# IST-DASLab/qutlass

Measured on AMD Instinct MI355X. Metric: TFLOP/s & %FP4-MFMA-peak, MXFP4 GEMM 4096x4096x4096, 1 MI355X, higher is better.
Workload: dtype fp4 (e2m1 x e2m1, e8m0 block scales, fp32 accumulate, bf16 out); 1 GPU; matmul_mxf4_bf16_tn 4096x4096x4096, gs=32 e8m0 scales (BASELINE.json configs[1]); parallelism=single GPU, clock_ramp=8200 untimed steps (~250 ms) before the 5 warmup steps

## Files before the change

qutlass_amd/csrc/capi.hip:

```cpp
#include <hip/hip_runtime.h>

#include <algorithm>
#include <atomic>
#include <chrono>
#include <cmath>
#include <cstdarg>
#include <cstdio>
#include <cstring>

#include "../../include/qutlass_amd.h"
#include "gemm_mx.hip.h"
#include "gemm_mx_deepp.hip.h"
#if QAMD_BENCH
#include "lab/gemm_mx_duo.hip.h"
#include "lab/gemm_mx_deepp_lab.hip.h"
#endif
#include "gemm_mx_skinny.hip.h"
#include "gemm_mx_ks.hip.h"
#include "gemm_mx_os.hip.h"
#include "gemm_mx_os_w4a8.hip.h"
#include "gemm_mx_fusedq.hip.h"
#include "gemm_nvf4.hip.h"
#include "gemm_nvf4_pk.hip.h"
#include "gemm_nvf4_os.hip.h"
#include "quantize.hip.h"
#include "moe_route.hip.h"
#include "to_blocked.hip.h"
#include "transpose_u8.hip.h"
#include "quartet_bwd.hip.h"
#if QAMD_BENCH
#include "lab/quartet_bwd_lab.hip.h"
#endif

using namespace qamd;

#ifndef QAMD_TU
#define QAMD_TU 0
#endif
#define QAMD_DEF(n) (QAMD_TU == 0 || QAMD_TU == (n))
#ifndef QAMD_BENCH
#define QAMD_BENCH 0
#endif

namespace qamd_host {

#if QAMD_DEF(1)
thread_local char g_err[512] = "";
#if QAMD_BENCH
std::atomic<int> g_hw_fp4_cvt{1};
std::atomic<int> g_gemm_variant{0};
std::atomic<int> g_nvf4_variant{0};
std::atomic<int> g_splitk_wg{0};
std::atomic<int> g_splitk_min_kt{32};
std::atomic<int> g_transpose_nc{0};
std::atomic<int> g_pp_shift{2};
std::atomic<int> g_pp_flags{1};
std::atomic<int> g_quant_wg_per_cu{0};
std::atomic<int> g_deepp_grid{0};
std::atomic<int> g_bwd_variant{0};
std::atomic<int> g_moe_sort_one_launch_max{0};
std::atomic<int> g_splitk_force{0};
std::atomic<uint32_t*> g_dbg{nullptr};
#endif

int fail(int code, const char* fmt, ...) {
  va_list ap;
  va_start(ap, fmt);
  vsnprintf(g_err, sizeof(g_err), fmt, ap);
  va_end(ap);
  return code;
}

int check_launch(const char* what) {
  hipError_t e = hipGetLastError();
  if (e != hipSuccess) return fail(QAMD_ERR_HIP, "%s: %s", what, hipGetErrorString(e));
  return QAMD_OK;
}

unsigned long long next_launch_tag() {
  static std::atomic<unsigned long long> tag{[] {
    unsigned long long x = (unsigned long long)std::chrono::steady_clock::now().time_since_epoch().count() ^ ((unsigned long long)(uintptr_t)&g_err << 17);
    x ^= x >> 31; x *= 0x9e3779b97f4a7c15ull; x ^= x >> 29;
    return x | 1ull;
  }()};
  return tag.fetch_add(1, std::memory_order_relaxed) + 1;
}
#else
unsigned long long next_launch_tag();
#if QAMD_BENCH
extern std::atomic<int> g_hw_fp4_cvt, g_gemm_variant, g_nvf4_variant, g_splitk_wg, g_splitk_min_kt, g_transpose_nc, g_pp_shift, g_pp_flags, g_quant_wg_per_cu, g_splitk_force, g_deepp_grid, g_bwd_variant, g_moe_sort_one_launch_max;
extern std::atomic<uint32_t*> g_dbg;
#endif
int fail(int code, const char* fmt, ...);
int check_launch(const char* what);
#endif

#if QAMD_BENCH
inline bool opt_hw_fp4() { return g_hw_fp4_cvt.load() != 0; }
inline int opt_gemm_variant() { return g_gemm_variant.load(); }
inline int opt_nvf4_variant() { return g_nvf4_variant.load(); }
inline int opt_splitk_wg() { return g_splitk_wg.load(); }
inline int opt_splitk_min_kt() { return g_splitk_min_kt.load(); }
inline int opt_transpose_nc() { return g_transpose_nc.load(); }
inline int opt_pp_shift() { return g_pp_shift.load(); }
inline int opt_pp_flags() { return g_pp_flags.load(); }
inline int opt_quant_wg_per_cu() { return g_quant_wg_per_cu.load(); }
inline int opt_splitk_force() { return g_splitk_force.load(); }
inline int opt_deepp_grid() { return g_deepp_grid.load(); }
inline int opt_bwd_variant() { return g_bwd_variant.load(); }
inline int opt_moe_sort_one_launch_max() { return g_moe_sort_one_launch_max.load(); }
inline uint32_t* opt_dbg() { return g_dbg.load(); }
#else
constexpr bool opt_hw_fp4() { return true; }
constexpr int opt_gemm_variant() { return 0; }
constexpr int opt_nvf4_variant() { return 0; }
constexpr int opt_splitk_wg() { return 0; }
constexpr int opt_splitk_min_kt() { return 32; }
constexpr int opt_transpose_nc() { return 0; }
constexpr int opt_pp_shift() { return 2; }
constexpr int opt_pp_flags() { return 1; }
constexpr int opt_quant_wg_per_cu() { return 0; }
constexpr int opt_splitk_force() { return 0; }
constexpr int opt_deepp_grid() { return 0; }
constexpr int opt_bwd_variant() { return 0; }
constexpr int opt_moe_sort_one_launch_max() { return 0; }
constexpr uint32_t* opt_dbg() { return nullptr; }
#endif

inline int64_t cdiv(int64_t a, int64_t b) { return (a + b - 1) / b; }

#if QAMD_DEF(1)
int chip_cus() {
  static std::atomic<int> cache[64];
  int dev = 0;
  if (hipGetDevice(&dev) != hipSuccess || dev < 0 || dev >= 64) return 256;
  int v = cache[dev].load(std::memory_order_relaxed);
  if (v <= 0) {
    int n = 0;
    if (hipDeviceGetAttribute(&n, hipDeviceAttributeMultiprocessorCount, dev) != hipSuccess || n <= 0) n = 256;
    cache[dev].store(n, std::memory_order_relaxed);
    v = n;
  }
  return v;
}
#else
int chip_cus();
#endif


template <class C, int PP>
int launch_gemm(GemmParams p, hipStream_t s) {
  p.tiles_m = (int)cdiv(p.M, C::BM);
  p.tiles_n = (int)cdiv(p.N, C::BN);
  p.raster_magic = raster_magic(p.tiles_n);
  if (PP != 7 && PP != 9) { p.ws = nullptr; p.splits = 1; p.ctr = nullptr; p.tag = 0; }
  hipLaunchKernelGGL((gemm_mx_kernel<C, PP>), dim3(p.tiles_m * p.tiles_n, p.splits), dim3(C::THREADS), 0, s, p);
  return check_launch("gemm_mx_kernel");
}

inline int deepp_grid(int tiles) {
  const int forced = opt_deepp_grid();
  if (forced > 0) return std::min(forced, tiles);
  const int cus = chip_cus();
  const int rounds = (tiles + cus - 1) / cus;
  const int g = ((tiles + rounds - 1) / rounds + 7) / 8 * 8;
  return std::min(std::min(g, cus), tiles);
}

template <class C, bool TRACE = false, int ST_AUX = 0, int LAB = 0>
int launch_gemm_deepp(GemmParams p, hipStream_t s) {
  p.tiles_m = (int)cdiv(p.M, C::BM);
  p.tiles_n = (int)cdiv(p.N, C::BN);
  p.raster_magic = raster_magic(p.tiles_n);
  p.ws = nullptr; p.splits = 1; p.ctr = nullptr; p.tag = 0;
  const int grid = deepp_grid(p.tiles_m * p.tiles_n);
#if QAMD_BENCH
#ifdef QAMD_ROUTE_LABK
  if constexpr (!TRACE && LAB == 0) {
    hipLaunchKernelGGL((labk::gemm_mx_deepp_kernel<C, false, ST_AUX, 8>), dim3(grid), dim3(C::THREADS), 0, s, p);
    return check_launch("labk::gemm_mx_deepp_kernel");
  }
#endif
  if constexpr (TRACE || LAB != 0) {
    hipLaunchKernelGGL((labk::gemm_mx_deepp_kernel<C, TRACE, ST_AUX, LAB>), dim3(grid), dim3(C::THREADS), 0, s, p);
    return check_launch("labk::gemm_mx_deepp_kernel");
  }
#else
  static_assert(!TRACE && LAB == 0, "traces / ablations: lab build only");
#endif
  const int64_t kt = cdiv((int64_t)p.K * C::EBITS / 8, 128);
  const bool odd = (kt & 1) && kt >= 3, one = grid == p.tiles_m * p.tiles_n;
  if (odd && one) hipLaunchKernelGGL((gemm_mx_deepp_kernel<C, ST_AUX, true, true>), dim3(grid), dim3(C::THREADS), 0, s, p);
  else if (odd) hipLaunchKernelGGL((gemm_mx_deepp_kernel<C, ST_AUX, true, false>), dim3(grid), dim3(C::THREADS), 0, s, p);
  else if (one) hipLaunchKernelGGL((gemm_mx_deepp_kernel<C, ST_AUX, false, true>), dim3(grid), dim3(C::THREADS), 0, s, p);
  else hipLaunchKernelGGL((gemm_mx_deepp_kernel<C, ST_AUX>), dim3(grid), dim3(C::THREADS), 0, s, p);
  return check_launch("gemm_mx_deepp_kernel");
}

#if QAMD_BENCH
template <class C, int ST_AUX = 17, int RET = 0, bool TRACE = false>
int launch_gemm_duo(GemmParams p, hipStream_t s) {
  p.tiles_m = (int)cdiv(p.M, C::BM);
  p.tiles_n = (int)cdiv(p.N, C::BN);
  p.raster_magic = raster_magic(p.tiles_n);
  p.ws = nullptr; p.splits = 1; p.ctr = nullptr; p.tag = 0;
  const int grid = deepp_grid(p.tiles_m * p.tiles_n);
  hipLaunchKernelGGL((gemm_mx_duo_kernel<C, ST_AUX, RET, TRACE>), dim3(grid), dim3(C::THREADS), 0, s, p);
  return check_launch("gemm_mx_duo_kernel");
}
#endif

template <int TM, int TN, int D = 8>
int launch_gemm_ks(GemmParams p, hipStream_t s) {
  using C = KsCfg<TM, TN, D>;
  p.tiles_m = (int)cdiv(p.M, TM);
  p.tiles_n = (int)cdiv(p.N, TN);
  p.ws = nullptr; p.splits = 1; p.ctr = nullptr; p.tag = 0;
  hipLaunchKernelGGL((gemm_mx_ks_kernel<C>), dim3(p.tiles_m * p.tiles_n), dim3(256), 0, s, p);
  return check_launch("gemm_mx_ks_kernel");
}

template <bool RM = false, int TN = 32, int EBITS = 4, int TM = 32, int AFMT = 0>
int launch_gemm_os(GemmParams p, hipStream_t s) {
  p.tiles_m = (int)cdiv(p.M, TM);
  p.tiles_n = (int)cdiv(p.N, TN);
  p.ws = nullptr; p.splits = 1; p.ctr = nullptr; p.tag = 0;
  const int64_t KT = cdiv((int64_t)p.K * EBITS / 8, 128);
  const dim3 grid(p.tiles_m * p.tiles_n), block(256);
  constexpr int SMAX = TM == 32 ? 4 : 3;
  if (KT <= 4) hipLaunchKernelGGL((gemm_mx_os_kernel<OsCfg<1, TN, EBITS, TM, AFMT>, RM>), grid, block, 0, s, p);
  else if (KT <= 8) hipLaunchKernelGGL((gemm_mx_os_kernel<OsCfg<2, TN, EBITS, TM, AFMT>, RM>), grid, block, 0, s, p);
  else if (KT <= 12) hipLaunchKernelGGL((gemm_mx_os_kernel<OsCfg<3, TN, EBITS, TM, AFMT>, RM>), grid, block, 0, s, p);
  else if (KT <= 4 * SMAX) hipLaunchKernelGGL((gemm_mx_os_kernel<OsCfg<SMAX, TN, EBITS, TM, AFMT>, RM>), grid, block, 0, s, p);
  else hipLaunchKernelGGL((gemm_mx_os_kernel<OsCfg<SMAX, TN, EBITS, TM, AFMT>, RM, true>), grid, block, 0, s, p);
  return check_launch("gemm_mx_os_kernel");
}
template <int EBITS = 4, int AFMT = 0, bool RM = false, int TN = 16>
int launch_gemm_os16(GemmParams p, hipStream_t s) {
  p.tiles_m = (int)cdiv(p.M, 16);
  p.tiles_n = (int)cdiv(p.N, TN);
  p.ws = nullptr; p.splits = 1; p.ctr = nullptr; p.tag = 0;
  const int64_t KT = cdiv((int64_t)p.K * EBITS / 8, 128);
  const dim3 grid(p.tiles_m * p.tiles_n), block(256);
  constexpr int STAGE = Os16Cfg<1, EBITS, AFMT, TN>::STAGE;
  constexpr int SFIT = 160 * 1024 / (4 * STAGE), SMAX = SFIT >= 8 ? 8 : SFIT >= 4 ? 4 : SFIT;
  static_assert(SMAX >= 3, "LDS budget");
  if (KT <= 4) hipLaunchKernelGGL((gemm_mx_os16_kernel<Os16Cfg<1, EBITS, AFMT, TN>, false, RM>), grid, block, 0, s, p);
  else if (KT <= 8) hipLaunchKernelGGL((gemm_mx_os16_kernel<Os16Cfg<2, EBITS, AFMT, TN>, false, RM>), grid, block, 0, s, p);
  else if (KT <= 16 && SMAX >= 4) hipLaunchKernelGGL((gemm_mx_os16_kernel<Os16Cfg<(SMAX >= 4 ? 4 : SMAX), EBITS, AFMT, TN>, false, RM>), grid, block, 0, s, p);
  else if (KT <= 4 * SMAX) hipLaunchKernelGGL((gemm_mx_os16_kernel<Os16Cfg<SMAX, EBITS, AFMT, TN>, false, RM>), grid, block, 0, s, p);
  else hipLaunchKernelGGL((gemm_mx_os16_kernel<Os16Cfg<SMAX, EBITS, AFMT, TN>, true, RM>), grid, block, 0, s, p);
  return check_launch("gemm_mx_os16_kernel");
}
inline int os16_tn(int64_t N, int64_t cus) {
  for (int tn : {16, 32, 48, 56, 64})
    if (cdiv(N, tn) <= cus) return tn;
  return 0;
}
inline int os16_wide_plan(int ebits, int64_t N, int64_t K, int64_t cus) {
  const int tn = os16_tn(N, cus);
  const int64_t KT = cdiv(K * ebits / 8, 128);
  if (ebits == 4) {
    if (tn == 32) return (KT >= 12 && KT <= 32) ? 572 : 0;
    if (tn == 48) return (KT >= 8 && KT <= 24) ? 573 : 0;
    if (tn == 56) return (KT >= 8 && KT <= 16) ? 574 : 0;
    if (tn == 64) return (KT >= 8 && KT <= 16) ? 575 : 0;
    return 0;
  }
  if (tn == 32) return (KT >= 16 && KT <= 64) ? 572 : 0;
  if (tn == 48) return (KT >= 16 && KT <= 32) ? 573 : 0;
  return 0;
}
template <int EBITS, int AFMT, bool RM>
int launch_gemm_os16_tn(int tn, const GemmParams& p, hipStream_t s) {
  switch (tn) {
    case 16: return launch_gemm_os16<EBITS, AFMT, RM, 16>(p, s);
    case 32: return launch_gemm_os16<EBITS, AFMT, RM, 32>(p, s);
    case 48: return launch_gemm_os16<EBITS, AFMT, RM, 48>(p, s);
    case 56: return launch_gemm_os16<EBITS, AFMT, RM, 56>(p, s);
    case 64: return launch_gemm_os16<EBITS, AFMT, RM, 64>(p, s);
  }
  return fail(QAMD_ERR_INVALID, "gemm_mx_os16: no column tile of %d", tn);
}
inline int os_plan(int64_t M, int64_t N, int64_t K, int64_t cus, bool ada = false) {
  const int64_t T32 = cdiv(M, 32) * cdiv(N, 32), T16 = cdiv(M, 32) * cdiv(N, 16), KT = cdiv(K, 256);
  if (T32 > cus) return 0;
  const int tn = T16 <= cus ? 16 : 32;
  if (KT <= 16) return tn;
  if (KT <= 32) return 4 * T32 >= cus ? tn : 0;
  if (KT > 64 || 2 * T32 < cus) return 0;
  return (ada || M >= 8 || tn == 16) ? tn : 0;
}

inline bool os64_plan(int64_t M, int64_t N, int64_t K, int64_t cus, bool ada = false) {
  const int64_t T32 = cdiv(M, 32) * cdiv(N, 32), T64 = cdiv(M, 64) * cdiv(N, 32), KT = cdiv(K, 256);
  if (T32 <= cus || T64 > cus) return false;
  if (ada) return KT <= 64;
  return KT <= 12 || (KT >= 40 && KT <= 64) || (KT >= 32 && KT < 40 && T64 == cus && M <= 64);
}
inline int os8_plan(int64_t M, int64_t N, int64_t K, int64_t cus) {
  const int64_t T32 = cdiv(M, 32) * cdiv(N, 32), T16 = cdiv(M, 32) * cdiv(N, 16), T64 = cdiv(M, 64) * cdiv(N, 32), KT = cdiv(K, 128);
  if (M <= 16) {
    if (const int v = os16_wide_plan(8, N, K, cus)) return v;
  }
  if (T32 <= cus) {
    const int v = T16 <= cus ? 569 : 568;
    const int64_t G = T16 <= cus ? T16 : T32;
    const bool d16 = cdiv(M, 16) * cdiv(N, 16) <= cus;
    if (KT <= 40) return d16 ? 571 : v;
    if (4 * G < 3 * cus) return 0;
    if (KT <= 64) return d16 ? 571 : v;
    if (KT <= 128) return (M <= 32 || N >= 4096) ? v : 0;
    return (KT <= 256 && M <= 32) ? v : 0;
  }
  return (T64 <= cus && KT > 16 && KT <= 128) ? 570 : 0;
}

inline int grouped_plan(int64_t M, int64_t N, int64_t K, int64_t E, int cus) {
  (void)N; (void)cus;
  return (M <= 32 * E && K <= 1024) ? 590 : 593;
}
inline int64_t grouped_grid(const GroupedFormat& F, int v, int64_t M, int64_t N, int64_t E) {
  return grouped_workgroups(M, N, E, F.tile[v - F.form0].tm, F.tile[v - F.form0].tn);
}
template <const GroupedFormat& F, int I, int AFMT = 0>
int launch_grouped_os(GroupedParams q, hipStream_t s) {
  constexpr int TM = F.tile[I].tm, TN = F.tile[I].tn, EBITS = F.ebits;
  q.tiles_m = 1;
  q.tiles_n = (int)cdiv(q.N, TN);
  const int64_t KT = cdiv((int64_t)q.K * EBITS / 8, 128);
  const dim3 grid((int)grouped_workgroups(q.M, q.N, q.E, TM, TN)), block(256);
  constexpr int SMAX = TM == 32 ? 4 : 3;
  if (KT <= 4) hipLaunchKernelGGL((gemm_mx_os_kernel<OsCfg<1, TN, EBITS, TM, AFMT>, true, false, true>), grid, block, 0, s, q);
  else if (KT <= 8) hipLaunchKernelGGL((gemm_mx_os_kernel<OsCfg<2, TN, EBITS, TM, AFMT>, true, false, true>), grid, block, 0, s, q);
  else if (KT <= 12) hipLaunchKernelGGL((gemm_mx_os_kernel<OsCfg<3, TN, EBITS, TM, AFMT>, true, false, true>), grid, block, 0, s, q);
  else if (KT <= 4 * SMAX) hipLaunchKernelGGL((gemm_mx_os_kernel<OsCfg<SMAX, TN, EBITS, TM, AFMT>, true, false, true>), grid, block, 0, s, q);
  else hipLaunchKernelGGL((gemm_mx_os_kernel<OsCfg<SMAX, TN, EBITS, TM, AFMT>, true, true, true>), grid, block, 0, s, q);
  return check_launch("gemm_mx_os_kernel (grouped)");
}
template <const GroupedFormat& F, class C>
int launch_grouped_ring(GroupedParams q, hipStream_t s) {
  static_assert(C::BM == F.tile[3].tm && C::BN == F.tile[3].tn && C::EBITS == F.ebits, "the ring configuration is the format's fourth form");
  q.tiles_m = 1;
  q.tiles_n = (int)cdiv(q.N, C::BN);
  hipLaunchKernelGGL((gemm_mx_grouped_ring_kernel<C>), dim3((int)grouped_workgroups(q.M, q.N, q.E, C::BM, C::BN)), dim3(C::THREADS), 0, s, q);
  return check_launch("gemm_mx_grouped_ring_kernel");
}
// ... 92 lines not shown
  return check_launch("gemm_mx_deepp_kernel (stream-K)");
}
#endif

template <class C, bool NN = false, int NNABL = 0>
int launch_gemm_deepp8(GemmParams p, hipStream_t s) {
  p.tiles_m = (int)cdiv(p.M, C::BM);
  p.tiles_n = (int)cdiv(p.N, C::BN);
  p.raster_magic = raster_magic(p.tiles_n);
  p.ws = nullptr; p.splits = 1; p.ctr = nullptr; p.tag = 0;
  const int grid = deepp_grid(p.tiles_m * p.tiles_n);
#if QAMD_BENCH
  if constexpr (NNABL != 0) {
    hipLaunchKernelGGL((labk::gemm_mx_deepp8_kernel<C, 17, NN, NNABL>), dim3(grid), dim3(C::THREADS), 0, s, p);
    return check_launch("labk::gemm_mx_deepp8_kernel");
  }
#else
  static_assert(NNABL == 0, "ablations: lab build only");
#endif
  if (grid == p.tiles_m * p.tiles_n) hipLaunchKernelGGL((gemm_mx_deepp8_kernel<C, 17, NN, true>), dim3(grid), dim3(C::THREADS), 0, s, p);
  else hipLaunchKernelGGL((gemm_mx_deepp8_kernel<C, 17, NN>), dim3(grid), dim3(C::THREADS), 0, s, p);
  return check_launch("gemm_mx_deepp8_kernel");
}

template <class CB, class CT, int ST_AUX>
int launch_gemm_hetero(GemmParams p, hipStream_t s) {
  p.tiles_m = (int)cdiv(p.M, CB::BM);
  p.tiles_n = (int)cdiv(p.N, CB::BN);
  p.raster_magic = raster_magic(p.tiles_n);
  p.ws = nullptr; p.splits = 1; p.ctr = nullptr; p.tag = 0;
  const int T = p.tiles_m * p.tiles_n;
  const int forced = opt_deepp_grid();
  const int g_big = std::min(forced > 0 ? forced : chip_cus(), T);
  const int t_main = T / g_big * g_big;
  const int nsmall = 4 * (T - t_main);
  if (nsmall == 0) {
    if constexpr (CB::EBITS == 4) return launch_gemm_deepp<CB, false, ST_AUX>(p, s);
    else return launch_gemm_deepp8<CB>(p, s);
  }
  if constexpr (CB::EBITS == 4) {
    if (const int64_t kt = cdiv((int64_t)p.K, 256); (kt & 1) && kt >= 3) {
      hipLaunchKernelGGL((gemm_mx_hetero_kernel<CB, CT, ST_AUX, true>), dim3(g_big + nsmall), dim3(256), 0, s, p, g_big, t_main);
      return check_launch("gemm_mx_hetero_kernel (odd stage count)");
    }
  }
  hipLaunchKernelGGL((gemm_mx_hetero_kernel<CB, CT, ST_AUX>), dim3(g_big + nsmall), dim3(256), 0, s, p, g_big, t_main);
  return check_launch("gemm_mx_hetero_kernel");
}

inline bool hetero_wins(int64_t T, int cus) {
  const int64_t r = T / cus, rem = T % cus;
  if (r < 1 || rem == 0) return false;
  const int64_t R = r + 1;
  const double a = (double)R * std::max(0.45 + 0.55 * (double)T / (double)(R * cus), 0.78);
  const int64_t nsmall = 4 * rem, waves = nsmall / cus;
  const double last = (double)(nsmall % cus) / (double)cus;
  const double b = (double)r + 0.05 + 0.38 * (double)waves + (last > 0 ? 0.25 + 0.13 * last : 0.0);
  return b < a;
}

#if QAMD_BENCH
#if QAMD_DEF(6)
int dispatch_ablation_mx4(int v, const GemmParams& p, hipStream_t s) {
  switch (v) {
#define QAMD_ABL(b) \
    case 100 + b: return launch_gemm<GemmCfg<256, 256, 2, 4, 4, false, b>, 1>(p, s); \
    case 200 + b: return launch_gemm<GemmCfg<256, 256, 2, 4, 4, false, b>, 0>(p, s); \
    case 300 + b: return launch_gemm<GemmCfg<256, 256, 2, 4, 4, false, b>, 2>(p, s);
    QAMD_ABL(1) QAMD_ABL(2) QAMD_ABL(3) QAMD_ABL(4) QAMD_ABL(8) QAMD_ABL(9) QAMD_ABL(10) QAMD_ABL(11) QAMD_ABL(16) QAMD_ABL(17) QAMD_ABL(18) QAMD_ABL(41) QAMD_ABL(40) QAMD_ABL(42)
#undef QAMD_ABL
  }
  return -1;
}
#else
int dispatch_ablation_mx4(int v, const GemmParams& p, hipStream_t s);
#endif
#endif

template <int EBITS, bool SPLIT>
int dispatch_variant(int v, const GemmParams& p, hipStream_t s, const char* name) {
#if QAMD_BENCH
  if (p.pp_flags & 4096) {
    if (v >= 70 && v <= 73) v += 100;
    else if (v == 24 || v == 25 || (v >= 27 && v <= 29)) v += 200;
  }
#endif
  switch (v) {
    case 24: return launch_gemm<GemmCfg<128, 128, 2, 2, EBITS, SPLIT, 0, 2>, 9>(p, s);
    case 25: return launch_gemm<GemmCfg<256, 128, 4, 2, EBITS, SPLIT, 0, 2>, 9>(p, s);
    case 27: return launch_gemm<GemmCfg<128, 64, 2, 2, EBITS, SPLIT, 0, 2>, 9>(p, s);
    case 58: return launch_gemm<GemmCfg<256, 128, 2, 2, EBITS, SPLIT, 0, 3>, 9>(p, s);
    case 28: return launch_gemm<GemmCfg<64, 128, 2, 2, EBITS, SPLIT, 0, 2>, 9>(p, s);
    case 29: return launch_gemm<GemmCfg<64, 64, 2, 2, EBITS, SPLIT, 0, 2>, 9>(p, s);
    case 70: return launch_gemm<GemmCfg<64, 64, 2, 2, EBITS, SPLIT, 0, 3>, 9>(p, s);
    case 71: return launch_gemm<GemmCfg<128, 64, 2, 2, EBITS, SPLIT, 0, 3>, 9>(p, s);
    case 72: return launch_gemm<GemmCfg<64, 128, 2, 2, EBITS, SPLIT, 0, 3>, 9>(p, s);
    case 73: return launch_gemm<GemmCfg<128, 128, 2, 2, EBITS, SPLIT, 0, 3>, 9>(p, s);
#if QAMD_BENCH
    case 273: return launch_gemm<GemmCfg<128, 128, 2, 2, EBITS, SPLIT, 128, 3>, 9>(p, s);
    case 272: return launch_gemm<GemmCfg<64, 128, 2, 2, EBITS, SPLIT, 128, 3>, 9>(p, s);
    case 270: return launch_gemm<GemmCfg<64, 64, 2, 2, EBITS, SPLIT, 128, 3>, 9>(p, s);
    case 224 + 1000: return launch_gemm<GemmCfg<128, 128, 2, 2, EBITS, SPLIT, 128, 2>, 9>(p, s);
    case 373: return launch_gemm<GemmCfg<128, 128, 2, 4, EBITS, SPLIT, 0, 3>, 9>(p, s);
    case 374: return launch_gemm<GemmCfg<128, 128, 4, 2, EBITS, SPLIT, 0, 3>, 9>(p, s);
    case 325: return launch_gemm<GemmCfg<256, 128, 2, 2, EBITS, SPLIT, 0, 3>, 9>(p, s);
    case 326: return launch_gemm<GemmCfg<128, 256, 2, 2, EBITS, SPLIT, 0, 3>, 9>(p, s);
    case 327: return launch_gemm<GemmCfg<256, 128, 2, 2, EBITS, SPLIT, 0, 2>, 9>(p, s);
    case 76: return launch_gemm<GemmCfg<128, 128, 2, 2, EBITS, SPLIT, 0, 4>, 9>(p, s);
    case 79: return launch_gemm<GemmCfg<64, 128, 2, 2, EBITS, SPLIT, 0, 4>, 9>(p, s);
    case 224: return launch_gemm<GemmCfg<128, 128, 2, 2, EBITS, SPLIT>, 3>(p, s);
    case 225: return launch_gemm<GemmCfg<256, 128, 4, 2, EBITS, SPLIT>, 3>(p, s);
    case 227: return launch_gemm<GemmCfg<128, 64, 2, 2, EBITS, SPLIT>, 3>(p, s);
    case 228: return launch_gemm<GemmCfg<64, 128, 2, 2, EBITS, SPLIT>, 3>(p, s);
    case 229: return launch_gemm<GemmCfg<64, 64, 2, 2, EBITS, SPLIT>, 3>(p, s);
    case 170: return launch_gemm<GemmCfg<64, 64, 2, 2, EBITS, SPLIT, 0, 3>, 7>(p, s);
    case 171: return launch_gemm<GemmCfg<128, 64, 2, 2, EBITS, SPLIT, 0, 3>, 7>(p, s);
    case 172: return launch_gemm<GemmCfg<64, 128, 2, 2, EBITS, SPLIT, 0, 3>, 7>(p, s);
    case 173: return launch_gemm<GemmCfg<128, 128, 2, 2, EBITS, SPLIT, 0, 3>, 7>(p, s);
    case 1: return launch_gemm<GemmCfg<256, 256, 2, 4, EBITS, SPLIT>, 1>(p, s);
    case 2: return launch_gemm<GemmCfg<128, 128, 2, 2, EBITS, SPLIT>, 0>(p, s);
    case 3: return launch_gemm<GemmCfg<256, 128, 4, 2, EBITS, SPLIT>, 0>(p, s);
    case 4: return launch_gemm<GemmCfg<128, 256, 2, 4, EBITS, SPLIT>, 0>(p, s);
    case 5: return launch_gemm<GemmCfg<256, 256, 2, 4, EBITS, SPLIT>, 0>(p, s);
    case 20: return launch_gemm<GemmCfg<256, 256, 2, 4, EBITS, SPLIT>, 3>(p, s);
    case 26: return launch_gemm<GemmCfg<128, 256, 2, 4, EBITS, SPLIT>, 3>(p, s);
    case 74: return launch_gemm<GemmCfg<64, 64, 2, 2, EBITS, SPLIT, 0, 4>, 7>(p, s);
    case 75: return launch_gemm<GemmCfg<64, 64, 2, 2, EBITS, SPLIT, 0, 6>, 7>(p, s);
    case 80: return launch_gemm<GemmCfg<64, 64, 2, 2, EBITS, SPLIT, 1, 3>, 7>(p, s);
    case 81: return launch_gemm<GemmCfg<64, 64, 2, 2, EBITS, SPLIT, 2, 3>, 7>(p, s);
    case 82: return launch_gemm<GemmCfg<64, 64, 2, 2, EBITS, SPLIT, 32, 3>, 7>(p, s);
    case 83: return launch_gemm<GemmCfg<64, 64, 2, 2, EBITS, SPLIT, 34, 3>, 7>(p, s);
    case 84: return launch_gemm<GemmCfg<64, 64, 2, 2, EBITS, SPLIT, 35, 3>, 7>(p, s);
    case 78: return launch_gemm<GemmCfg<64, 64, 2, 2, EBITS, SPLIT, 16, 3>, 7>(p, s);
#endif
  }
  if constexpr (EBITS == 8) {
#if QAMD_BENCH
    if (v == 89) return launch_gemm_deepp_sk<GemmCfg<256, 256, 2, 2, 8, true>>(p, s);
#endif
    if (v == 90) return launch_gemm_deepp8<GemmCfg<256, 256, 2, 2, 8, true>>(p, s);
    if (v == 568) return launch_gemm_os<false, 32, 8>(p, s);
    if (v == 569) return launch_gemm_os<false, 16, 8>(p, s);
    if (v == 570) return launch_gemm_os<false, 32, 8, 64>(p, s);
    if (v >= 571 && v <= 575) return launch_gemm_os16_tn<8, 0, false>(v == 571 ? 16 : v == 572 ? 32 : v == 573 ? 48 : v == 574 ? 56 : 64, p, s);
    if (v == 98) return launch_gemm_hetero<GemmCfg<256, 256, 2, 2, 8, true>, GemmCfg<128, 128, 2, 2, 8, true, 0, 4>, 17>(p, s);
#if QAMD_BENCH
    if (v == 30) return launch_gemm<GemmCfg<256, 256, 2, 2, 8, true>, 4>(p, s);
#endif
  }
  if constexpr (EBITS == 4) {
#if QAMD_BENCH
    if (v == 89) return launch_gemm_deepp_sk<GemmCfg<256, 256, 2, 2, 4, false>>(p, s);
#endif
    if (v == 90) return launch_gemm_deepp<GemmCfg<256, 256, 2, 2, 4, false>, false, 17>(p, s);
    if (v == 98) return launch_gemm_hetero<GemmCfg<256, 256, 2, 2, 4, false>, GemmCfg<128, 128, 2, 2, 4, false, 0, 4>, 17>(p, s);
    if (v == 561 || v == 562) {
      const bool deep = cdiv(p.K, 256) > 24;
      if (v == 561) return deep ? launch_gemm_ks<32, 32, 6>(p, s) : launch_gemm_ks<32, 32, 4>(p, s);
      return deep ? launch_gemm_ks<32, 64, 6>(p, s) : launch_gemm_ks<32, 64, 4>(p, s);
    }
    if (v == 568) return launch_gemm_os<false>(p, s);
    if (v == 569) return launch_gemm_os<false, 16>(p, s);
    if (v == 570) return launch_gemm_os<false, 32, 4, 64>(p, s);
    if (v >= 571 && v <= 575) return launch_gemm_os16_tn<4, 0, false>(v == 571 ? 16 : v == 572 ? 32 : v == 573 ? 48 : v == 574 ? 56 : 64, p, s);
#if QAMD_BENCH
    if (v == 99) return launch_gemm_hetero<GemmCfg<256, 256, 2, 2, 4, false>, GemmCfg<128, 128, 2, 2, 4, false, 0, 3>, 17>(p, s);
    if (v == 563 || v == 564) {
      const bool deep = cdiv(p.K, 256) > 24;
      if (v == 563) return deep ? launch_gemm_ks<64, 32, 6>(p, s) : launch_gemm_ks<64, 32, 4>(p, s);
      return deep ? launch_gemm_ks<64, 64, 6>(p, s) : launch_gemm_ks<64, 64, 4>(p, s);
    }
    if (v == 565) return launch_gemm_ks<32, 32, 4>(p, s);
    if (v == 566) return launch_gemm_ks<32, 32, 8>(p, s);
    if (v == 567) return launch_gemm_ks<32, 32, 6>(p, s);
    if (v == 88) return launch_gemm_duo<GemmCfg<256, 256, 2, 4, 4, false>, 17, 0>(p, s);
    if (v == 87) return launch_gemm_duo<GemmCfg<256, 256, 2, 4, 4, false>, 17, 1>(p, s);
    if (v == 86) return launch_gemm_duo<GemmCfg<256, 256, 2, 4, 4, false>, 17, 0, true>(p, s);
    if (v == 298) return launch_gemm_hetero<GemmCfg<256, 256, 2, 2, 4, false>, GemmCfg<128, 128, 2, 2, 4, false, 128, 4>, 17>(p, s);
    if (v == 91) return launch_gemm_deepp<GemmCfg<256, 256, 2, 2, 4, false>, true, 17>(p, s);
    if (v == 92) return launch_gemm_deepp<GemmCfg<256, 256, 2, 2, 4, false>, false, 2>(p, s);
    if (v == 93) return launch_gemm_deepp<GemmCfg<256, 256, 2, 2, 4, false>, false, 16>(p, s);
    if (v == 94) return launch_gemm_deepp<GemmCfg<256, 256, 2, 2, 4, false>, false, 0>(p, s);
    if (v == 95) return launch_gemm_deepp<GemmCfg<256, 256, 2, 2, 4, false>, false, 19>(p, s);
    if (v == 96) return launch_gemm_deepp<GemmCfg<256, 256, 2, 2, 4, false>, false, 1>(p, s);
    if (v == 97) return launch_gemm_deepp<GemmCfg<256, 256, 2, 2, 4, false>, false, 17, 1>(p, s);
    if (v == 197) return launch_gemm_deepp<GemmCfg<256, 256, 2, 2, 4, false>, false, 17, 2>(p, s);
    if (v == 297) return launch_gemm_deepp<GemmCfg<256, 256, 2, 2, 4, false>, false, 17, 3>(p, s);
    if (v == 397) return launch_gemm_deepp<GemmCfg<256, 256, 2, 2, 4, false>, false, 17, 4>(p, s);
    switch (v) {
      case 6: return launch_gemm<GemmCfg<256, 256, 2, 4, 4, false>, 2>(p, s);
      case 7: return launch_gemm<GemmCfg<128, 128, 2, 2, 4, false>, 2>(p, s);
      case 8: return launch_gemm<GemmCfg<256, 128, 4, 2, 4, false>, 2>(p, s);
      case 9: return launch_gemm<GemmCfg<128, 256, 2, 4, 4, false>, 2>(p, s);
      case 30: return launch_gemm<GemmCfg<256, 256, 2, 2, 4, false>, 4>(p, s);
      case 31: return launch_gemm<GemmCfg<256, 256, 2, 2, 4, false, 8>, 4>(p, s);
      case 32: return launch_gemm<GemmCfg<256, 256, 2, 2, 4, false, 9>, 4>(p, s);
      case 33: return launch_gemm<GemmCfg<256, 256, 2, 2, 4, false, 10>, 4>(p, s);
      case 34: return launch_gemm<GemmCfg<256, 256, 2, 2, 4, false, 40>, 4>(p, s);
      case 40: return launch_gemm<GemmCfg<256, 256, 2, 2, 4, false>, 5>(p, s);
      case 41: return launch_gemm<GemmCfg<256, 256, 2, 2, 4, false, 8>, 5>(p, s);
      case 42: return launch_gemm<GemmCfg<256, 256, 2, 2, 4, false, 9>, 5>(p, s);
      case 43: return launch_gemm<GemmCfg<256, 256, 2, 2, 4, false, 10>, 5>(p, s);
      case 50: return launch_gemm<GemmCfg<256, 256, 2, 4, 4, false, 64>, 3>(p, s);
      case 51: return launch_gemm<GemmCfg<256, 256, 2, 2, 4, false, 64>, 4>(p, s);
      case 52: return launch_gemm<GemmCfg<256, 256, 2, 2, 4, false, 64>, 5>(p, s);
      case 53: return launch_gemm<GemmCfg<256, 256, 2, 2, 4, false, 72>, 5>(p, s);
      case 54: return launch_gemm<GemmCfg<256, 256, 2, 2, 4, false, 73>, 5>(p, s);
      case 55: return launch_gemm<GemmCfg<256, 256, 2, 2, 4, false, 74>, 5>(p, s);
      case 56: return launch_gemm<GemmCfg<256, 256, 2, 2, 4, false, 104>, 5>(p, s);
      case 35: return launch_gemm<GemmCfg<256, 256, 2, 2, 4, false, 16>, 4>(p, s);
      case 36: return launch_gemm<GemmCfg<256, 256, 2, 2, 4, false, 17>, 4>(p, s);
      case 21: return launch_gemm<GemmCfg<256, 256, 2, 4, 4, false, 8>, 3>(p, s);
      case 22: return launch_gemm<GemmCfg<256, 256, 2, 4, 4, false, 9>, 3>(p, s);
      case 23: return launch_gemm<GemmCfg<256, 256, 2, 4, 4, false, 10>, 3>(p, s);
    }
#endif
  }
#if QAMD_BENCH
  if constexpr (EBITS == 4 && !SPLIT) {
    const int rc = dispatch_ablation_mx4(v, p, s);
    if (rc >= 0) return rc;
  }
#endif
  return fail(QAMD_ERR_INVALID, "%s: unknown gemm_variant %d", name, v);
}

int dispatch_variant_a5(int v, const GemmParams& p, hipStream_t s, const char* name)
#if QAMD_DEF(4)
{
  switch (v) {
    case 24: return launch_gemm<GemmCfg<128, 128, 2, 2, 8, true, 0, 2, 1>, 9>(p, s);
    case 25: return launch_gemm<GemmCfg<256, 128, 4, 2, 8, true, 0, 2, 1>, 9>(p, s);
    case 27: return launch_gemm<GemmCfg<128, 64, 2, 2, 8, true, 0, 2, 1>, 9>(p, s);
    case 58: return launch_gemm<GemmCfg<256, 128, 2, 2, 8, true, 0, 3, 1>, 9>(p, s);
    case 28: return launch_gemm<GemmCfg<64, 128, 2, 2, 8, true, 0, 2, 1>, 9>(p, s);
    case 29: return launch_gemm<GemmCfg<64, 64, 2, 2, 8, true, 0, 2, 1>, 9>(p, s);
    case 90: return launch_gemm_deepp8<GemmCfg<256, 256, 2, 2, 8, true, 0, 2, 1>>(p, s);
    case 98: return launch_gemm_hetero<GemmCfg<256, 256, 2, 2, 8, true, 0, 2, 1>, GemmCfg<128, 128, 2, 2, 8, true, 0, 4, 1>, 17>(p, s);
    case 70: return launch_gemm<GemmCfg<64, 64, 2, 2, 8, true, 0, 3, 1>, 9>(p, s);
    case 71: return launch_gemm<GemmCfg<128, 64, 2, 2, 8, true, 0, 3, 1>, 9>(p, s);
    case 72: return launch_gemm<GemmCfg<64, 128, 2, 2, 8, true, 0, 3, 1>, 9>(p, s);
    case 73: return launch_gemm<GemmCfg<128, 128, 2, 2, 8, true, 0, 3, 1>, 9>(p, s);
    case 568: return launch_gemm_os<false, 32, 8, 32, 1>(p, s);
    case 569: return launch_gemm_os<false, 16, 8, 32, 1>(p, s);
    case 570: return launch_gemm_os<false, 32, 8, 64, 1>(p, s);
    case 571: case 572: case 573: case 574: case 575: return launch_gemm_os16_tn<8, 1, false>(v == 571 ? 16 : v == 572 ? 32 : v == 573 ? 48 : v == 574 ? 56 : 64, p, s);
  }
  return fail(QAMD_ERR_INVALID, "%s: gemm_variant %d has no e5m2-operand instantiation", name, v);
}
int launch_nn_fused_a5(const GemmParams& p, hipStream_t s, bool per_tile) {
#if QAMD_BENCH
  if (per_tile) return launch_gemm<GemmCfg<256, 256, 2, 2, 8, true, 0, 2, 1>, 6>(p, s);
#endif
  (void)per_tile;
  return launch_gemm_deepp8<GemmCfg<256, 256, 2, 2, 8, true, 0, 2, 1>, true>(p, s);
}
#else
;
int launch_nn_fused_a5(const GemmParams& p, hipStream_t s, bool per_tile);
#endif

#if QAMD_TU != 0
#if QAMD_TU == 2
template int dispatch_variant<4, false>(int, const GemmParams&, hipStream_t, const char*);
#else
extern template int dispatch_variant<4, false>(int, const GemmParams&, hipStream_t, const char*);
#endif
#if QAMD_TU == 3
template int dispatch_variant<8, true>(int, const GemmParams&, hipStream_t, const char*);
#if QAMD_BENCH
template int launch_gemm<GemmCfg<256, 256, 2, 2, 8, true>, 6>(GemmParams, hipStream_t);
#endif
#else
extern template int dispatch_variant<8, true>(int, const GemmParams&, hipStream_t, const char*);
#if QAMD_BENCH
extern template int launch_gemm<GemmCfg<256, 256, 2, 2, 8, true>, 6>(GemmParams, hipStream_t);
#endif
#endif
#endif

#if QAMD_DEF(4)
int launch_nvf4_host(const NvLaunch& l, const NvGemmParams& p, hipStream_t s) { return launch_nvf4_gemm(l, p, s) == hipSuccess ? 0 : 1; }
int launch_nvf4_grouped_host(const NvGroupedParams& q, hipStream_t s, int form) { return launch_nvf4_grouped(q, s, form) == hipSuccess ? 0 : 1; }
#else
int launch_nvf4_host(const NvLaunch& l, const NvGemmParams& p, hipStream_t s);
int launch_nvf4_grouped_host(const NvGroupedParams& q, hipStream_t s, int form);
#endif

#if QAMD_DEF(1)
struct SmallPlan { int variant; int splits; };
inline void ring_tile(int variant, int& bm, int& bn) {
  bm = (variant == 71 || variant == 73) ? 128 : 64;
  bn = (variant == 72 || variant == 73) ? 128 : 64;
}
inline int64_t splitk_partial_bytes(int64_t M, int64_t N, int splits) { return (int64_t)splits * M * N * 4; }
inline int64_t splitk_ctr_offset(int64_t M, int64_t N, int splits) { return (splitk_partial_bytes(M, N, splits) + 255) / 256 * 256; }
inline int64_t splitk_ws_bytes(int variant, int64_t M, int64_t N, int splits) {
#if QAMD_BENCH
  int bm, bn;
  ring_tile(variant, bm, bn);
  return splitk_ctr_offset(M, N, splits) + cdiv(M, bm) * cdiv(N, bn) * 8;
#else
  (void)variant;
  return splitk_partial_bytes(M, N, splits);
#endif
}
template <int EBITS>
SmallPlan plan_small_rule(int64_t M, int64_t N, int64_t K, int64_t cus, bool may_split) {
  const int64_t T64 = cdiv(M, 64) * cdiv(N, 64), T128 = cdiv(M, 128) * cdiv(N, 128);
  if (T64 <= cus) {
    const int64_t KT = cdiv(K * EBITS / 8, 128);
    int64_t S = 1;
    if (may_split && T64 < cus && KT >= opt_splitk_min_kt()) {
      const int64_t wg = opt_splitk_wg() > 0 ? opt_splitk_wg() : cus;
      S = std::min<int64_t>(std::min<int64_t>(8, wg / T64), KT / 8);
      if (S < 1) S = 1;
      const int64_t per = cdiv(KT, S);
      S = cdiv(KT, per);
      if (S == 2 && KT < 48) S = 1;
    }
    return {70, (int)S};
  }
  if (T64 <= 2 * cus) return {N >= M ? 72 : 71, 1};
  if (M > 64 && N > 64 && T128 <= cus) return {73, 1};
  return {0, 1};
}

template <int EBITS>
SmallPlan plan_small(int64_t M, int64_t N, int64_t K, int64_t cus, bool may_split) {
  const SmallPlan cur = plan_small_rule<EBITS>(M, N, K, cus, may_split);
  if (cur.variant != 70 && cur.variant != 72 && cur.variant != 73) return cur;
// ... 1488 lines not shown
```

Baseline: 4563 TFLOP/s.

## Add specialized one-tile-per-CTA deep-pipelined MXFP4 kernel with 16x16x128 MFMA schedule

Adds a new kernel for the case where each CTA owns exactly one 256x256 tile. It uses the 16x16x128 scaled MFMA with a hand-interleaved schedule of fragment reads, scale shifts and DMA issue. The final stage overlaps the epilogue (scratch write, read and bf16 store) with the last MFMAs, row by row, to hide the tail. This path is the default for the one-tile case; forced variants for A/B comparison exist in lab builds only. The hand schedule risks register pressure and instruction-issue hazards.

```diff
diff --git a/qutlass_amd/csrc/capi.hip b/qutlass_amd/csrc/capi.hip
--- a/qutlass_amd/csrc/capi.hip
+++ b/qutlass_amd/csrc/capi.hip
@@ -11,6 +11,7 @@
 #include "../../include/qutlass_amd.h"
 #include "gemm_mx.hip.h"
 #include "gemm_mx_deepp.hip.h"
+#include "gemm_mx_deepp16.hip.h"
 #if QAMD_BENCH
 #include "lab/gemm_mx_duo.hip.h"
 #include "lab/gemm_mx_deepp_lab.hip.h"
@@ -167,7 +168,7 @@
   return std::min(std::min(g, cus), tiles);
 }
 
-template <class C, bool TRACE = false, int ST_AUX = 0, int LAB = 0>
+template <class C, bool TRACE = false, int ST_AUX = 0, int LAB = 0, int ONEFORM = 0>
 int launch_gemm_deepp(GemmParams p, hipStream_t s) {
   p.tiles_m = (int)cdiv(p.M, C::BM);
   p.tiles_n = (int)cdiv(p.N, C::BN);
@@ -192,7 +193,12 @@
   const bool odd = (kt & 1) && kt >= 3, one = grid == p.tiles_m * p.tiles_n;
   if (odd && one) hipLaunchKernelGGL((gemm_mx_deepp_kernel<C, ST_AUX, true, true>), dim3(grid), dim3(C::THREADS), 0, s, p);
   else if (odd) hipLaunchKernelGGL((gemm_mx_deepp_kernel<C, ST_AUX, true, false>), dim3(grid), dim3(C::THREADS), 0, s, p);
-  else if (one) hipLaunchKernelGGL((gemm_mx_deepp_kernel<C, ST_AUX, false, true>), dim3(grid), dim3(C::THREADS), 0, s, p);
+  else if (one) {
+    static_assert(ONEFORM == 0 || ONEFORM == 16 || ONEFORM == 32, "one-tile form");
+    static_assert(ONEFORM == 0 || QAMD_BENCH, "forced one-tile forms: lab build only");
+    if constexpr (ONEFORM == 16 || (ONEFORM == 0 && kDeeppOneTile16)) hipLaunchKernelGGL((gemm_mx_deepp16_kernel<C, ST_AUX>), dim3(grid), dim3(C::THREADS), 0, s, p);
+    else hipLaunchKernelGGL((gemm_mx_deepp_kernel<C, ST_AUX, false, true>), dim3(grid), dim3(C::THREADS), 0, s, p);
+  }
   else hipLaunchKernelGGL((gemm_mx_deepp_kernel<C, ST_AUX>), dim3(grid), dim3(C::THREADS), 0, s, p);
   return check_launch("gemm_mx_deepp_kernel");
 }
@@ -591,7 +597,7 @@
 #if QAMD_BENCH
     if (v == 89) return launch_gemm_deepp_sk<GemmCfg<256, 256, 2, 2, 4, false>>(p, s);
 #endif
-    if (v == 90) return launch_gemm_deepp<GemmCfg<256, 256, 2, 2, 4, false>, false, 17>(p, s);
+    if (v == 90) return launch_gemm_deepp<GemmCfg<256, 256, 2, 2, 4, false>, false, 17, 0, QAMD_BENCH ? 32 : 0>(p, s);
     if (v == 98) return launch_gemm_hetero<GemmCfg<256, 256, 2, 2, 4, false>, GemmCfg<128, 128, 2, 2, 4, false, 0, 4>, 17>(p, s);
     if (v == 561 || v == 562) {
       const bool deep = cdiv(p.K, 256) > 24;
@@ -616,6 +622,8 @@
     if (v == 87) return launch_gemm_duo<GemmCfg<256, 256, 2, 4, 4, false>, 17, 1>(p, s);
     if (v == 86) return launch_gemm_duo<GemmCfg<256, 256, 2, 4, 4, false>, 17, 0, true>(p, s);
     if (v == 298) return launch_gemm_hetero<GemmCfg<256, 256, 2, 2, 4, false>, GemmCfg<128, 128, 2, 2, 4, false, 128, 4>, 17>(p, s);
+    if (v == 190) return launch_gemm_deepp<GemmCfg<256, 256, 2, 2, 4, false>, false, 17, 0, 32>(p, s);
+    if (v == 191) return launch_gemm_deepp<GemmCfg<256, 256, 2, 2, 4, false>, false, 17, 0, 16>(p, s);
     if (v == 91) return launch_gemm_deepp<GemmCfg<256, 256, 2, 2, 4, false>, true, 17>(p, s);
     if (v == 92) return launch_gemm_deepp<GemmCfg<256, 256, 2, 2, 4, false>, false, 2>(p, s);
     if (v == 93) return launch_gemm_deepp<GemmCfg<256, 256, 2, 2, 4, false>, false, 16>(p, s);
diff --git a/qutlass_amd/csrc/gemm_mx_deepp16.hip.h b/qutlass_amd/csrc/gemm_mx_deepp16.hip.h
--- /dev/null
+++ b/qutlass_amd/csrc/gemm_mx_deepp16.hip.h
@@ -0,0 +1,242 @@
+#pragma once
+#include "gemm_mx_deepp.hip.h"
+
+namespace qamd {
+
+constexpr bool kDeeppOneTile16 = true;
+
+constexpr int deepp16_row_done_at(int s) { return (s >= 7 && s <= 63 && (s - 7) % 8 == 0) ? (s - 7) / 8 : -1; }
+
+template <class C, int ST_AUX = 0>
+__device__ __forceinline__ void gemm_mx_deepp16(char* smem, const GemmParams& p, const int bid, const int G, const int ntiles) {
+  static_assert(C::EBITS == 4 && C::BM == 256 && C::BN == 256 && C::WAVES_M == 2 && C::WAVES_N == 2 && C::NSTAGE == 2 && C::PPW == 2,
+                "persistent deep schedule: fp4, 256x256 tiles, 4 waves of 128x128");
+  constexpr int MT = 8, NT = 8;
+  constexpr int STAGE = C::STAGE_BYTES, OFF_SCR = DeepPCfg<C>::OFF_SCR;
+  GemmCtx<C> cx(smem, p);
+  const int lane = cx.lane, wave = cx.wave, r16 = lane & 15, kq = lane >> 4;
+  const int KT = cx.KT, KTe = (KT + 1) & ~1, CB = cx.CB, rowbytes = cx.rowbytes;
+  const int tile = xcd_remap(bid, G);
+
+  auto fence = [&]() __attribute__((always_inline)) { __builtin_amdgcn_sched_barrier(0); };
+  struct Desc { __amdgpu_buffer_rsrc_t a, b, s; };
+  int m0, n0;
+  {
+    int tm, tn;
+    raster_decode(tile < ntiles ? tile : ntiles - 1, p.tiles_m, p.tiles_n, p.raster_magic, tm, tn);
+    m0 = uniform(tm * C::BM);
+    n0 = uniform(tn * C::BN);
+  }
+  Desc cur;
+  {
+    const bool valid = tile < ntiles;
+    const uint32_t a_off = (uint32_t)m0 * rowbytes, b_off = (uint32_t)n0 * rowbytes;
+    const uint32_t sa_off = (uint32_t)(m0 >> 7) * CB * 512, sb_off = (uint32_t)(n0 >> 7) * CB * 512;
+    cur.a = make_rsrc(p.A + a_off, valid ? p.a_bytes - a_off : 0u);
+    cur.b = make_rsrc(p.B + b_off, valid ? p.b_bytes - b_off : 0u);
+    cur.s = cx.sIsB ? make_rsrc(p.SFB + sb_off, valid ? p.sfb_bytes - sb_off : 0u) : make_rsrc(p.SFA + sa_off, valid ? p.sfa_bytes - sa_off : 0u);
+  }
+
+  v4f acc[MT][NT];
+  v4i fa[2][MT], fb[2][NT];
+  v4i xq[2][4];
+  const int sh = 8 * kq;
+
+  const int sw = (r16 >> 1) & 7;
+  int rdF[2];
+#pragma unroll
+  for (int h = 0; h < 2; ++h) rdF[h] = (cx.wave_m * C::WTM + r16) * C::ROWB + (((4 * h + kq) ^ sw) << 4);
+  const int rdBd = cx.rdBd;
+  const int rdSA = C::OFF_S + (cx.wave_m * C::SCT) * 512 + r16 * 16, rdSB = C::OFF_S + (C::PA + cx.wave_n * C::SCT) * 512 + r16 * 16;
+  static_assert(C::SCT == 2 && C::WTM == 128 && C::WTN == 128, "a wave's rows are one 128-row scale tile; a stage is two column tiles");
+
+  typedef __attribute__((address_space(3))) const v4i* lds_v4i_t;
+  uint32_t rbA = 0, rbB = 0;
+  auto read_base = [&](const int buf, const int h) __attribute__((always_inline)) {
+    rbA = (uint32_t)(uintptr_t)(lds_ptr_t)(smem + buf * STAGE + rdF[h]);
+    rbB = rbA + (uint32_t)rdBd;
+    asm volatile("" : "+v"(rbA), "+v"(rbB));
+  };
+  auto read_frag = [&](const int h, const int i) __attribute__((always_inline)) {
+    if (i < MT) fa[h][i] = *(lds_v4i_t)(uintptr_t)(rbA + (uint32_t)(i * 16 * C::ROWB));
+    else fb[h][i - MT] = *(lds_v4i_t)(uintptr_t)(rbB + (uint32_t)((i - MT) * 16 * C::ROWB));
+  };
+  auto read_raw = [&](const int buf, const int h, const int k) __attribute__((always_inline)) {
+    xq[h][k] = *(const v4i*)(smem + buf * STAGE + (k < 2 ? rdSA : rdSB) + h * 512 + (k & 1) * 256);
+  };
+  auto shift1 = [&](const int h, const int k) __attribute__((always_inline)) {
+    xq[h][k >> 2][k & 3] = (int)((unsigned)xq[h][k >> 2][k & 3] >> sh);
+  };
+  auto mfma1 = [&](const int h, const int m, const int n, const bool zero_c) __attribute__((always_inline)) {
+    const v4i a = fa[h][m], b = fb[h][n];
+    const int sb1 = xq[h][2 + (n & 1)][n >> 1], sa1 = xq[h][m & 1][m >> 1];
+    if (zero_c)
+      asm volatile("v_mfma_scale_f32_16x16x128_f8f6f4 %0, %1, %2, 0, %3, %4 op_sel_hi:[0,0,0] cbsz:4 blgp:4" : "=a"(acc[m][n]) : "v"(b), "v"(a), "v"(sb1), "v"(sa1));
+    else
+      asm volatile("v_mfma_scale_f32_16x16x128_f8f6f4 %0, %1, %2, %0, %3, %4 op_sel_hi:[0,0,0] cbsz:4 blgp:4" : "+a"(acc[m][n]) : "v"(b), "v"(a), "v"(sb1), "v"(sa1));
+  };
+
+  int vb0 = 0, vb1 = 0, vbS = 0;
+  auto dma_prep = [&](int kt, bool valid) __attribute__((always_inline)) {
+    int lastmask = (kt == KT - 1) ? -1 : 0;
+    int oobm = (valid && kt < KT) ? 0 : -1;
+    int oobs = (valid && kt * C::SCT + cx.colS < CB) ? 0 : -1;
+    asm volatile("" : "+v"(lastmask), "+v"(oobm), "+v"(oobs));
+    vb0 = (((cx.voffT[0] & lastmask) | (cx.voffAB[0] & ~lastmask)) & ~oobm) | ((int)0x80000000 & oobm);
+    vb1 = (((cx.voffT[1] & lastmask) | (cx.voffAB[1] & ~lastmask)) & ~oobm) | ((int)0x80000000 & oobm);
+    vbS = (cx.voffS & ~oobs) | ((int)0x80000000 & oobs);
+  };
+  auto dma_item = [&](const Desc& d, int kt, const int buf, const int item) __attribute__((always_inline)) {
+    char* st = smem + buf * STAGE;
+    if (item < 16) {
+      const int t = item & 7, q = wave * 8 + t;
+      const int v = ((t & 1) ? vb1 : vb0) + q * cx.rstep;
+      __builtin_amdgcn_raw_ptr_buffer_load_lds(item < 8 ? d.a : d.b, (lds_ptr_t)(st + (item < 8 ? 0 : C::OFF_B) + q * 1024), 16, v, kt * C::ROWB, 0, QAMD_DMA_AUX);
+    } else {
+      __builtin_amdgcn_raw_ptr_buffer_load_lds(d.s, (lds_ptr_t)(st + C::OFF_S + wave * 1024), 16, vbS, kt * C::SCT * 512, 0, 0);
+    }
+  };
+  auto dma_stage = [&](const Desc& d, int kt, bool valid, const int buf) __attribute__((always_inline)) {
+    dma_prep(kt, valid);
+#pragma unroll
+    for (int i = 0; i < 17; ++i) dma_item(d, kt, buf, i);
+  };
+
+  auto half = [&](const int h, const bool zero_c, auto extra) __attribute__((always_inline)) {
+    int i = 0;
+#pragma unroll
+    for (int m = 0; m < MT; ++m)
+#pragma unroll
+      for (int n = 0; n < NT; ++n) {
+        mfma1(h, m, n, zero_c);
+        extra(i);
+        fence();
+        ++i;
+      }
+  };
+  auto fill = [&](const int buf, const int hs, const int i) __attribute__((always_inline)) {
+    if (i < 32 && (i & 1)) read_frag(hs, i >> 1);
+    if (i >= 33 && i < 40 && (i & 1)) read_raw(buf, hs, (i - 33) >> 1);
+    if (i >= 46 && i < 62) shift1(hs, i - 46);
+  };
+
+  auto stage = [&](auto bufc, auto firstc, int ktl, bool dvalid, auto dmac) __attribute__((always_inline)) {
+    constexpr int BUF = decltype(bufc)::value;
+    constexpr bool FIRST = decltype(firstc)::value;
+    constexpr bool DMA = decltype(dmac)::value;
+    read_base(BUF, 1);
+    half(0, FIRST, [&](const int i) __attribute__((always_inline)) {
+      fill(BUF, 1, i);
+      if (DMA && i == 42) dma_prep(ktl, dvalid);
+      if (i == 63) read_base(BUF ^ 1, 0);
+    });
+    asm volatile("s_waitcnt vmcnt(0) lgkmcnt(0)" ::: "memory");
+    __builtin_amdgcn_s_barrier();
+    fence();
+    half(1, false, [&](const int i) __attribute__((always_inline)) {
+      fill(BUF ^ 1, 0, i);
+      if (DMA && !(i & 1) && i < 34) dma_item(cur, ktl, BUF, i >> 1);
+    });
+  };
+
+  char* scr = smem + OFF_SCR + wave * DeepPCfg<C>::SCR_PER_WAVE;
+  const int scrW = r16 * 512 + ((kq ^ (r16 & 7)) << 4);
+  const int rrl = lane >> 3, ccl = lane & 7;
+  const int scrR = rrl * 512 + (ccl >> 2) * 128 + ((((2 * ccl) & 7) ^ rrl) << 4);
+  const float alpha = *p.alpha;
+  __amdgpu_buffer_rsrc_t rD;
+  int stLane, colLim;
+  {
+    const int64_t left = ((int64_t)(p.M - m0) * p.ldd - n0) * 2;
+    rD = make_rsrc(p.D + ((int64_t)m0 * p.ldd + n0), (uint32_t)(left > 0x7fffffffll ? 0x7fffffffll : left));
+    stLane = ((cx.wave_m * C::WTM + rrl) * p.ldd + cx.wave_n * C::WTN + 8 * ccl) * 2;
+    colLim = p.N - n0 - cx.wave_n * C::WTN - 8 * ccl;
+  }
+  auto retire_write = [&](const int m) __attribute__((always_inline)) {
+    asm volatile("s_nop 15" ::: "memory");
+#pragma unroll
+    for (int n = 0; n < NT; ++n) *(v4f*)(scr + (scrW ^ ((n & 1) << 6)) + (n >> 1) * 128) = acc[m][n];
+  };
+  v4f rb[2][2];
+  auto retire_read = [&](const int rh) __attribute__((always_inline)) {
+#pragma unroll
+    for (int ch = 0; ch < 2; ++ch) {
+      rb[ch][0] = *(const v4f*)(scr + scrR + rh * 4096 + ch * 256);
+      rb[ch][1] = *(const v4f*)(scr + (scrR ^ 16) + rh * 4096 + ch * 256);
+    }
+  };
+  auto retire_store = [&](const int m, const int pass) __attribute__((always_inline)) {
+    const int rh = pass >> 1, ch = pass & 1;
+    const v4f lo = rb[ch][0], hi = rb[ch][1];
+    v4i o;
+    o[0] = (int)pack_bf16x2(lo[0] * alpha, lo[1] * alpha);
+    o[1] = (int)pack_bf16x2(lo[2] * alpha, lo[3] * alpha);
+    o[2] = (int)pack_bf16x2(hi[0] * alpha, hi[1] * alpha);
+    o[3] = (int)pack_bf16x2(hi[2] * alpha, hi[3] * alpha);
+    int ldd2 = p.ldd * 2;
+    asm volatile("" : "+s"(ldd2));
+    __builtin_amdgcn_raw_buffer_store_b128(__builtin_bit_cast(v4u, o), rD, (64 * ch < colLim) ? stLane : (int)0x80000000, (16 * m + 8 * rh) * ldd2 + 128 * ch, ST_AUX);
+  };
+
+  auto final_stage = [&]() __attribute__((always_inline)) {
+    read_base(1, 1);
+    half(0, false, [&](const int i) __attribute__((always_inline)) { fill(1, 1, i); });
+    asm volatile("s_waitcnt vmcnt(0) lgkmcnt(0)" ::: "memory");
+    __builtin_amdgcn_s_barrier();
+    fence();
+    static_for<0, 75>([&](auto sc) __attribute__((always_inline)) {
+      constexpr int s = decltype(sc)::value;
+      if constexpr (s < 64) mfma1(1, s / 8, s % 8, false);
+      constexpr int d1 = s - 1, d3 = s - 3, d5 = s - 5, d6 = s - 6, d7 = s - 7, d9 = s - 9, d10 = s - 10;
+      if constexpr (deepp16_row_done_at(d5) >= 0) retire_store(deepp16_row_done_at(d5), 0);
+      if constexpr (deepp16_row_done_at(d6) >= 0) retire_store(deepp16_row_done_at(d6), 1);
+      if constexpr (deepp16_row_done_at(d9) >= 0) retire_store(deepp16_row_done_at(d9), 2);
+      if constexpr (deepp16_row_done_at(d10) >= 0) retire_store(deepp16_row_done_at(d10), 3);
+      if constexpr (deepp16_row_done_at(d1) >= 0) retire_write(deepp16_row_done_at(d1));
+      if constexpr (deepp16_row_done_at(d3) >= 0) retire_read(0);
+      if constexpr (deepp16_row_done_at(d7) >= 0) retire_read(1);
+      fence();
+    });
+  };
+
+  using I0 = std::integral_constant<int, 0>;
+  using I1 = std::integral_constant<int, 1>;
+  using BT = std::integral_constant<bool, true>;
+  using BF = std::integral_constant<bool, false>;
+
+  dma_stage(cur, 0, true, 0);
+  dma_stage(cur, 1, true, 1);
+  asm volatile("s_waitcnt vmcnt(17)" ::: "memory");
+  __builtin_amdgcn_s_barrier();
+  fence();
+#pragma unroll
+  for (int k = 0; k < 4; ++k) read_raw(0, 0, k);
+  read_base(0, 0);
+#pragma unroll
+  for (int i = 0; i < MT + NT; ++i) read_frag(0, i);
+#pragma unroll
+  for (int k = 0; k < 16; ++k) shift1(0, k);
+  fence();
+
+  stage(I0{}, BT{}, 2, true, BT{});
+  int kt = 1;
+  for (; kt + 4 < KTe; kt += 2) {
+    stage(I1{}, BF{}, kt + 2, true, BT{});
+    stage(I0{}, BF{}, kt + 3, true, BT{});
+  }
+  if (kt + 2 < KTe) {
+    stage(I1{}, BF{}, kt + 2, true, BT{});
+    stage(I0{}, BF{}, 0, false, BF{});
+  }
+  final_stage();
+  asm volatile("s_waitcnt vmcnt(0)" ::: "memory");
+}
+
+template <class C, int ST_AUX = 0>
+__global__ __launch_bounds__(C::THREADS) void gemm_mx_deepp16_kernel(const GemmParams p) {
+  __shared__ __attribute__((aligned(16))) char smem[DeepPCfg<C>::LDS_BYTES];
+  asm volatile("" :: "s"(p.A), "s"(p.D), "s"(p.K), "s"(p.b_bytes), "s"((int)gridDim.x));
+  gemm_mx_deepp16<C, ST_AUX>(smem, p, (int)blockIdx.x, (int)gridDim.x, p.tiles_m * p.tiles_n);
+}
+
+}
```

Measured after the change: 4679 TFLOP/s, median of 6. +2.5%, better.
